# Lain-Iwakuro/Plonky2-Demo

Hardware: NVIDIA B200
Metric: lde_merkle_commit_elems_per_s (higher is better)
Workload: dtype u64 (Goldilocks field, integer)

## Files before the change

### plonky2_demo_b200/csrc/poseidon.cuh

```cuda
#pragma once
#include "gl64.cuh"
#include "poseidon_constants.cuh"

namespace pcs {

#ifndef PCS_MDS_FP64
#define PCS_MDS_FP64 1
#endif
#ifndef PCS_SBOX_GROUP
#define PCS_SBOX_GROUP 12
#endif

constexpr int SPONGE_WIDTH = 12;
constexpr int SPONGE_RATE = 8;

__device__ __forceinline__ uint64_t sbox7(uint64_t x) {
    uint64_t x2 = gl::sqr(x);
    uint64_t x4 = gl::sqr(x2);
    uint64_t x3 = gl::mul(x, x2);
    return gl::mul(x3, x4);
}

__device__ __forceinline__ void mds_half(const uint32_t (&s)[12], const uint32_t (&add)[12], uint64_t (&y)[12]) {
    int64_t A[3], B[3], P[3], Q[3];
#pragma unroll
    for (int j = 0; j < 3; j++) {
        int64_t s0 = s[j], s3 = s[j + 3], s6 = s[j + 6], s9 = s[j + 9];
        int64_t u = s0 + s6, v = s3 + s9;
        A[j] = u + v;
        B[j] = u - v;
        P[j] = s0 - s6;
        Q[j] = s3 - s9;
    }
    int64_t t = A[0] + A[1] + A[2];
    int64_t Ya[3] = {(t + A[2]) << 4, (t + A[0]) << 4, (t + A[1]) << 4};
    int64_t Yb[3] = {(B[2] << 3) - (B[1] << 1) - B[0],
                     -(B[0] << 3) - B[1] - (B[2] << 1),
                     (B[0] << 1) - (B[1] << 3) - B[2]};
    int64_t re[3], im[3];
    re[0] = (P[0] << 1) - Q[0] + P[1] - (Q[1] << 4) + P[2] + (Q[2] << 2);
    im[0] = P[0] + (Q[0] << 1) + (P[1] << 4) + Q[1] - (P[2] << 2) + Q[2];
    re[1] = -(P[0] << 2) + Q[0] + (P[1] << 1) - Q[1] + P[2] - (Q[2] << 4);
    im[1] = -P[0] - (Q[0] << 2) + P[1] + (Q[1] << 1) + (P[2] << 4) + Q[2];
    re[2] = (P[0] << 4) + Q[0] - (P[1] << 2) + Q[1] + (P[2] << 1) - Q[2];
    im[2] = -P[0] + (Q[0] << 4) - P[1] - (Q[1] << 2) + P[2] + (Q[2] << 1);
#pragma unroll
    for (int j = 0; j < 3; j++) {
        int64_t e1 = Ya[j] + Yb[j], e2 = Ya[j] - Yb[j];
        y[j] = (uint64_t)(e1 + re[j] + (int64_t)add[j]);
        y[j + 3] = (uint64_t)(e2 + im[j] + (int64_t)add[j + 3]);
        y[j + 6] = (uint64_t)(e1 - re[j] + (int64_t)add[j + 6]);
        y[j + 9] = (uint64_t)(e2 - im[j] + (int64_t)add[j + 9]);
    }
    y[0] += (uint64_t)s[0] << 3;
}

template <int RC_MODE >
__device__ __forceinline__ void mds_layer(uint64_t (&s)[12], const uint64_t* __restrict__ rc) {
    uint32_t lo[12], hi[12], alo[12], ahi[12];
#pragma unroll
    for (int i = 0; i < 12; i++) {
        lo[i] = (uint32_t)s[i];
        hi[i] = (uint32_t)(s[i] >> 32);
        uint64_t c = (RC_MODE == 1 || (RC_MODE == 2 && i == 0)) ? rc[i] : 0;
        alo[i] = (uint32_t)c;
        ahi[i] = (uint32_t)(c >> 32);
    }
    uint64_t L[12], H[12];
    mds_half(lo, alo, L);
    mds_half(hi, ahi, H);
#pragma unroll
    for (int r = 0; r < 12; r++) s[r] = gl::fold_halves(L[r], H[r]);
}

constexpr double TWO52 = 4503599627370496.0;

__device__ __forceinline__ void mds_half_fp64(const uint32_t (&s)[12], const double* __restrict__ addb ,
                                              uint32_t (&ylo)[12], uint32_t (&yhi)[12]) {
    double A[3], B[3], P[3], Q[3];
    double s0d;
#pragma unroll
    for (int j = 0; j < 3; j++) {
        double v0 = __hiloint2double(0x43300000, (int)s[j]), v3 = __hiloint2double(0x43300000, (int)s[j + 3]);
        double v6 = __hiloint2double(0x43300000, (int)s[j + 6]), v9 = __hiloint2double(0x43300000, (int)s[j + 9]);
        double d6 = v6 - TWO52, d9 = v9 - TWO52;
        P[j] = v0 - v6;
        Q[j] = v3 - v9;
        double u = fma(d6, 2.0, P[j]);
        double v = fma(d9, 2.0, Q[j]);
        A[j] = u + v;
        B[j] = u - v;
        if (j == 0) s0d = P[0] + d6;
    }
    double t = A[0] + A[1] + A[2];
    double Ya[3] = {t + A[2], t + A[0], t + A[1]};
    double Yb[3] = {fma(B[1], -2.0, fma(B[2], 8.0, -B[0])),
                    fma(B[2], -2.0, fma(B[0], -8.0, -B[1])),
                    fma(B[1], -8.0, fma(B[0], 2.0, -B[2]))};
    double re[3], im[3];
    re[0] = fma(Q[2], 4.0, fma(Q[1], -16.0, fma(P[0], 2.0, -Q[0]) + P[1]) + P[2]);
    im[0] = fma(P[2], -4.0, fma(P[1], 16.0, fma(Q[0], 2.0, P[0]) + Q[1]) + Q[2]);
    re[1] = fma(Q[2], -16.0, fma(P[1], 2.0, fma(P[0], -4.0, Q[0]) - Q[1]) + P[2]);
    im[1] = fma(P[2], 16.0, fma(Q[1], 2.0, fma(Q[0], -4.0, -P[0]) + P[1]) + Q[2]);
    re[2] = fma(P[2], 2.0, fma(P[1], -4.0, fma(P[0], 16.0, Q[0]) + Q[1]) - Q[2]);
    im[2] = fma(Q[2], 2.0, fma(Q[1], -4.0, fma(Q[0], 16.0, -P[0]) - P[1]) + P[2]);
#pragma unroll
    for (int j = 0; j < 3; j++) {
        double e1 = fma(Ya[j], 16.0, Yb[j]), e2 = fma(Ya[j], 16.0, -Yb[j]);
        double y0 = e1 + re[j];
        if (j == 0) y0 = fma(s0d, 8.0, y0);
        double r0 = y0 + addb[2 * j];
        double r3 = (e2 + im[j]) + addb[2 * (j + 3)];
        double r6 = (e1 - re[j]) + addb[2 * (j + 6)];
        double r9 = (e2 - im[j]) + addb[2 * (j + 9)];
        ylo[j] = (uint32_t)__double2loint(r0);     yhi[j] = (uint32_t)__double2hiint(r0);
        ylo[j + 3] = (uint32_t)__double2loint(r3); yhi[j + 3] = (uint32_t)__double2hiint(r3);
        ylo[j + 6] = (uint32_t)__double2loint(r6); yhi[j + 6] = (uint32_t)__double2hiint(r6);
        ylo[j + 9] = (uint32_t)__double2loint(r9); yhi[j + 9] = (uint32_t)__double2hiint(r9);
    }
}

__device__ __forceinline__ void mds_layer_fp64(uint64_t (&s)[12], const uint64_t* __restrict__ rcd) {
    const double* addb = reinterpret_cast<const double*>(rcd);
    uint32_t lo[12], hi[12];
#pragma unroll
    for (int i = 0; i < 12; i++) {
        lo[i] = (uint32_t)s[i];
        hi[i] = (uint32_t)(s[i] >> 32);
    }
    uint32_t l0[12], l1[12], h0[12], h1[12];
    mds_half_fp64(lo, addb, l0, l1);
    mds_half_fp64(hi, addb + 1, h0, h1);
#pragma unroll
    for (int r = 0; r < 12; r++) s[r] = gl::fold_halves_biased(l0[r], l1[r], h0[r], h1[r]);
}

__device__ __forceinline__ double u32_as_double(uint32_t x) { return __hiloint2double(0x43300000, (int)x) - TWO52; }

template <bool ZERO0>
__device__ __forceinline__ void mds_net_d(const double (&s)[12], double (&y)[12]) {
    double A[3], B[3], P[3], Q[3];
#pragma unroll
    for (int j = 0; j < 3; j++) {
        const bool z = ZERO0 && j == 0;
        double u = z ? s[6] : s[j] + s[j + 6], v = s[j + 3] + s[j + 9];
        A[j] = u + v;
        B[j] = u - v;
        P[j] = z ? -s[6] : s[j] - s[j + 6];
        Q[j] = s[j + 3] - s[j + 9];
    }
    double t = A[0] + A[1] + A[2];
    double Ya[3] = {t + A[2], t + A[0], t + A[1]};
    double Yb[3] = {fma(B[1], -2.0, fma(B[2], 8.0, -B[0])),
                    fma(B[2], -2.0, fma(B[0], -8.0, -B[1])),
                    fma(B[1], -8.0, fma(B[0], 2.0, -B[2]))};
    double re[3], im[3];
    re[0] = fma(Q[2], 4.0, fma(Q[1], -16.0, fma(P[0], 2.0, -Q[0]) + P[1]) + P[2]);
    im[0] = fma(P[2], -4.0, fma(P[1], 16.0, fma(Q[0], 2.0, P[0]) + Q[1]) + Q[2]);
    re[1] = fma(Q[2], -16.0, fma(P[1], 2.0, fma(P[0], -4.0, Q[0]) - Q[1]) + P[2]);
    im[1] = fma(P[2], 16.0, fma(Q[1], 2.0, fma(Q[0], -4.0, -P[0]) + P[1]) + Q[2]);
    re[2] = fma(P[2], 2.0, fma(P[1], -4.0, fma(P[0], 16.0, Q[0]) + Q[1]) - Q[2]);
    im[2] = fma(Q[2], 2.0, fma(Q[1], -4.0, fma(Q[0], 16.0, -P[0]) - P[1]) + P[2]);
#pragma unroll
    for (int j = 0; j < 3; j++) {
        double e1 = fma(Ya[j], 16.0, Yb[j]), e2 = fma(Ya[j], 16.0, -Yb[j]);
        y[j] = e1 + re[j];
        y[j + 3] = e2 + im[j];
        y[j + 6] = e1 - re[j];
        y[j + 9] = e2 - im[j];
    }
    if (!ZERO0) y[0] = fma(s[0], 8.0, y[0]);
}

__device__ __forceinline__ void renorm_d(double& lo, double& hi) {
    const double M1 = TWO52 + 1.0, INV32 = 1.0 / 4294967296.0;
    double l1m = __fma_rd(lo, INV32, TWO52) - M1;
    double h1m = __fma_rd(hi, INV32, TWO52) - M1;
    double lo2 = fma(l1m, -4294967296.0, lo) - h1m;
    double hi2 = fma(h1m, -4294967295.0, hi) + l1m;
    lo = lo2;
    hi = hi2;
}

__device__ __forceinline__ uint64_t fold_d(double lo, double hi) {
    double bl = lo + TWO52, bh = hi + TWO52;
    return gl::fold_halves_biased((uint32_t)__double2loint(bl), (uint32_t)__double2hiint(bl),
                                  (uint32_t)__double2loint(bh), (uint32_t)__double2hiint(bh));
}

#ifndef PCS_PARTIAL_SPLIT
#define PCS_PARTIAL_SPLIT 0
#endif
__device__ __forceinline__ void partial_round_d(uint64_t& x0, double (&dl)[12], double (&dh)[12], uint64_t rc) {
    double yl[12], yh[12];
#if PCS_PARTIAL_SPLIT
    mds_net_d<true>(dl, yl);
    mds_net_d<true>(dh, yh);
    x0 = gl::add_lc_p(sbox7(x0), rc);
    const double al = u32_as_double((uint32_t)x0), ah = u32_as_double((uint32_t)(x0 >> 32));
    constexpr double COL0[12] = {25.0, 20.0, 34.0, 18.0, 39.0, 13.0, 13.0, 28.0, 2.0, 16.0, 41.0, 15.0};
#pragma unroll
    for (int i = 0; i < 12; i++) {
        dl[i] = fma(al, COL0[i], yl[i]);
        dh[i] = fma(ah, COL0[i], yh[i]);
    }
#else
    x0 = gl::add_lc_p(sbox7(x0), rc);
    dl[0] = u32_as_double((uint32_t)x0);
    dh[0] = u32_as_double((uint32_t)(x0 >> 32));
    mds_net_d<false>(dl, yl);
    mds_net_d<false>(dh, yh);
#pragma unroll
    for (int i = 0; i < 12; i++) {
        dl[i] = yl[i];
        dh[i] = yh[i];
    }
#endif
}

#ifndef PCS_PARTIAL_FP64
#define PCS_PARTIAL_FP64 1
#endif

__device__ __forceinline__ void full_round(uint64_t (&s)[12], int r) {
    using namespace pconst;
#if PCS_SBOX_GROUP == 12
#pragma unroll
    for (int i = 0; i < 12; i++) s[i] = sbox7(s[i]);
#else
#pragma unroll 1
    for (int g = 0; g < 12 / PCS_SBOX_GROUP; g++) {
        uint64_t t[PCS_SBOX_GROUP];
#pragma unroll
        for (int i = 0; i < PCS_SBOX_GROUP; i++) t[i] = sbox7(s[i]);
#pragma unroll
        for (int i = 0; i < 12 - PCS_SBOX_GROUP; i++) s[i] = s[i + PCS_SBOX_GROUP];
#pragma unroll
        for (int i = 0; i < PCS_SBOX_GROUP; i++) s[12 - PCS_SBOX_GROUP + i] = t[i];
    }
#endif
#if PCS_MDS_FP64
    mds_layer_fp64(s, &ROUND_ADD_D[24 * r]);
#else
    mds_layer<1>(s, &ROUND_ADD[12 * r]);
#endif
}

template <bool CANON_OUT = true>
__device__ __forceinline__ void poseidon12(uint64_t (&s)[12]) {
    using namespace pconst;
#pragma unroll
    for (int i = 0; i < 12; i++) s[i] = gl::add_lc_p(s[i], RC[i]);
#if PCS_PARTIAL_FP64 && PCS_MDS_FP64
#pragma unroll 1
    for (int phase = 0; phase < 2; phase++) {
#pragma unroll 1
        for (int r = 0; r < 4; r++) full_round(s, 26 * phase + r);
        if (phase == 0) {
            uint64_t x0 = s[0];
            double dl[12], dh[12];
#pragma unroll
            for (int i = 1; i < 12; i++) {
                dl[i] = u32_as_double((uint32_t)s[i]);
                dh[i] = u32_as_double((uint32_t)(s[i] >> 32));
            }
#pragma unroll 1
            for (int k = 0; k < 11; k++) {
                partial_round_d(x0, dl, dh, PARTIAL_RC[2 * k]);
                x0 = fold_d(dl[0], dh[0]);
                partial_round_d(x0, dl, dh, PARTIAL_RC[2 * k + 1]);
                if (k < 10) {
                    x0 = fold_d(dl[0], dh[0]);
#pragma unroll
                    for (int i = 1; i < 12; i++) renorm_d(dl[i], dh[i]);
                }
            }
            const double* rcd = reinterpret_cast<const double*>(&ROUND_ADD_D[24 * 25]);
#pragma unroll
            for (int i = 0; i < 12; i++) {
                double bl = dl[i] + rcd[2 * i], bh = dh[i] + rcd[2 * i + 1];
                s[i] = gl::fold_halves_biased((uint32_t)__double2loint(bl), (uint32_t)__double2hiint(bl),
                                              (uint32_t)__double2loint(bh), (uint32_t)__double2hiint(bh));
            }
        }
    }
#else
#pragma unroll 1
    for (int r = 0; r < 30; r++) {
        if (r < 4 || r >= 26) {
#pragma unroll
            for (int i = 0; i < 12; i++) s[i] = sbox7(s[i]);
        } else {
            s[0] = sbox7(s[0]);
        }
#if PCS_MDS_FP64
        mds_layer_fp64(s, &ROUND_ADD_D[24 * r]);
#else
        mds_layer<1>(s, &ROUND_ADD[12 * r]);
#endif
    }
#endif
    if (CANON_OUT) {
#pragma unroll
        for (int i = 0; i < 12; i++) s[i] = gl::canon(s[i]);
    }
}

}
```

Baseline: 9.582 billion.

## Keep Poseidon partial-round state in a transformed (CRT-like) FP64 basis

Replaces the per-partial-round full MDS butterfly in FP64 with a state kept in a pre-transformed basis (forward/mid/scale stages). Each round then only updates lane 0 and runs a reduced mid-stage before converting back to output lanes at the end. Renormalization now uses a different magic constant that allows signed values, and a biased fold is applied to lane 0. The aim is fewer FP64 operations per partial round, at the cost of more intricate numeric range reasoning and a risk of exactness errors.

Measured after the change: 10.07 billion, median of 6. 5.1% higher.

```diff
diff --git a/plonky2_demo_b200/csrc/poseidon.cuh b/plonky2_demo_b200/csrc/poseidon.cuh
--- a/plonky2_demo_b200/csrc/poseidon.cuh
+++ b/plonky2_demo_b200/csrc/poseidon.cuh
@@ -136,6 +136,7 @@
 }
 
 __device__ __forceinline__ double u32_as_double(uint32_t x) { return __hiloint2double(0x43300000, (int)x) - TWO52; }
+__device__ __forceinline__ double u32_biased(uint32_t x) { return __hiloint2double(0x43300000, (int)x); }
 
 template <bool ZERO0>
 __device__ __forceinline__ void mds_net_d(const double (&s)[12], double (&y)[12]) {
@@ -172,50 +173,89 @@
     if (!ZERO0) y[0] = fma(s[0], 8.0, y[0]);
 }
 
+__device__ __forceinline__ void crt_forward_d(const uint32_t (&s)[12], double (&u)[12]) {
+#pragma unroll
+    for (int j = 0; j < 3; j++) {
+        double v0 = u32_biased(s[j]), v3 = u32_biased(s[j + 3]), v6 = u32_biased(s[j + 6]), v9 = u32_biased(s[j + 9]);
+        double P = v0 - v6, Q = v3 - v9;
+        double a = fma(v6 - TWO52, 2.0, P);
+        double b = fma(v9 - TWO52, 2.0, Q);
+        u[j] = a + b;
+        u[j + 3] = a - b;
+        u[j + 6] = P;
+        u[j + 9] = Q;
+    }
+}
+
+__device__ __forceinline__ void crt_mid_half(const double (&u)[12], double g, double (&w)[12]) {
+    const double A0 = u[0] + g, A1 = u[1], A2 = u[2];
+    const double B0 = u[3] + g, B1 = u[4], B2 = u[5];
+    const double P0 = u[6] + g, P1 = u[7], P2 = u[8];
+    const double Q0 = u[9], Q1 = u[10], Q2 = u[11];
+    const double T = ((A1 + A2) + A0) * 64.0;
+    w[0] = fma(A2, 64.0, T);
+    w[1] = fma(A0, 64.0, T);
+    w[2] = fma(A1, 64.0, T);
+    w[3] = fma(B1, -2.0, fma(B2, 8.0, -B0));
+    w[4] = fma(B2, -2.0, fma(B0, -8.0, -B1));
+    w[5] = fma(B1, -8.0, fma(B0, 2.0, -B2));
+    w[6] = fma(Q2, 4.0, fma(Q1, -16.0, fma(P0, 2.0, -Q0) + P1) + P2);
+    w[7] = fma(Q2, -16.0, fma(P1, 2.0, fma(P0, -4.0, Q0) - Q1) + P2);
+    w[8] = fma(P2, 2.0, fma(P1, -4.0, fma(P0, 16.0, Q0) + Q1) - Q2);
+    w[9] = fma(P2, -4.0, fma(P1, 16.0, fma(Q0, 2.0, P0) + Q1) + Q2);
+    w[10] = fma(P2, 16.0, fma(Q1, 2.0, fma(Q0, -4.0, -P0) + P1) + Q2);
+    w[11] = fma(Q2, 2.0, fma(Q1, -4.0, fma(Q0, 16.0, -P0) - P1) + P2);
+}
+
+__device__ __forceinline__ double crt_scale_half(const double (&w)[12], double (&u)[12]) {
+#pragma unroll
+    for (int j = 0; j < 3; j++) {
+        u[j] = w[j];
+        u[j + 3] = w[j + 3] * 4.0;
+        u[j + 6] = w[j + 6] * 2.0;
+        u[j + 9] = w[j + 9] * 2.0;
+    }
+    return fma(w[0], 0.25, w[3] + w[6]);
+}
+
+__device__ __forceinline__ void crt_lanes_half(const double (&w)[12], double bias, const double* __restrict__ rcd,
+                                               double (&y)[12]) {
+#pragma unroll
+    for (int j = 0; j < 3; j++) {
+        double e1 = fma(w[j], 0.25, w[j + 3] + bias), e2 = fma(w[j], 0.25, bias - w[j + 3]);
+        y[j] = (e1 + w[j + 6]) + rcd[2 * j];
+        y[j + 6] = (e1 - w[j + 6]) + rcd[2 * (j + 6)];
+        y[j + 3] = (e2 + w[j + 9]) + rcd[2 * (j + 3)];
+        y[j + 9] = (e2 - w[j + 9]) + rcd[2 * (j + 9)];
+    }
+}
+
 __device__ __forceinline__ void renorm_d(double& lo, double& hi) {
-    const double M1 = TWO52 + 1.0, INV32 = 1.0 / 4294967296.0;
-    double l1m = __fma_rd(lo, INV32, TWO52) - M1;
-    double h1m = __fma_rd(hi, INV32, TWO52) - M1;
-    double lo2 = fma(l1m, -4294967296.0, lo) - h1m;
-    double hi2 = fma(h1m, -4294967295.0, hi) + l1m;
+    const double C = 6755399441055744.0, INV32 = 1.0 / 4294967296.0;
+    double l1 = __fma_rd(lo, INV32, C) - C;
+    double h1 = __fma_rd(hi, INV32, C) - C;
+    double lo2 = fma(l1, -4294967296.0, lo) - h1;
+    double hi2 = fma(h1, -4294967295.0, hi) + l1;
     lo = lo2;
     hi = hi2;
 }
 
-__device__ __forceinline__ uint64_t fold_d(double lo, double hi) {
-    double bl = lo + TWO52, bh = hi + TWO52;
+constexpr double BIAS_LO = 2251799813685248.0 + 524288.0;
+constexpr double BIAS_HI = 2251799813685248.0 - 1048576.0;
+
+__device__ __forceinline__ uint64_t fold_signed_d(double lo, double hi) {
+    double bl = lo + (TWO52 + BIAS_LO), bh = hi + (TWO52 + BIAS_HI);
     return gl::fold_halves_biased((uint32_t)__double2loint(bl), (uint32_t)__double2hiint(bl),
                                   (uint32_t)__double2loint(bh), (uint32_t)__double2hiint(bh));
 }
 
-#ifndef PCS_PARTIAL_SPLIT
-#define PCS_PARTIAL_SPLIT 0
-#endif
-__device__ __forceinline__ void partial_round_d(uint64_t& x0, double (&dl)[12], double (&dh)[12], uint64_t rc) {
-    double yl[12], yh[12];
-#if PCS_PARTIAL_SPLIT
-    mds_net_d<true>(dl, yl);
-    mds_net_d<true>(dh, yh);
-    x0 = gl::add_lc_p(sbox7(x0), rc);
-    const double al = u32_as_double((uint32_t)x0), ah = u32_as_double((uint32_t)(x0 >> 32));
-    constexpr double COL0[12] = {25.0, 20.0, 34.0, 18.0, 39.0, 13.0, 13.0, 28.0, 2.0, 16.0, 41.0, 15.0};
-#pragma unroll
-    for (int i = 0; i < 12; i++) {
-        dl[i] = fma(al, COL0[i], yl[i]);
-        dh[i] = fma(ah, COL0[i], yh[i]);
-    }
-#else
-    x0 = gl::add_lc_p(sbox7(x0), rc);
-    dl[0] = u32_as_double((uint32_t)x0);
-    dh[0] = u32_as_double((uint32_t)(x0 >> 32));
-    mds_net_d<false>(dl, yl);
-    mds_net_d<false>(dh, yh);
-#pragma unroll
-    for (int i = 0; i < 12; i++) {
-        dl[i] = yl[i];
-        dh[i] = yh[i];
-    }
-#endif
+__device__ __forceinline__ void lane0_crt(double el, double eh, double& xl, double& xh, uint64_t rc, double& gl, double& gh) {
+    const uint64_t s0 = fold_signed_d(fma(xl, 8.0, el), fma(xh, 8.0, eh));
+    const uint64_t x = gl::add_lc_p(sbox7(s0), rc);
+    gl = fma(xl, 8.0, u32_biased((uint32_t)x) - u32_biased((uint32_t)s0));
+    gh = fma(xh, 8.0, u32_biased((uint32_t)(x >> 32)) - u32_biased((uint32_t)(s0 >> 32)));
+    xl = u32_as_double((uint32_t)x);
+    xh = u32_as_double((uint32_t)(x >> 32));
 }
 
 #ifndef PCS_PARTIAL_FP64
@@ -257,28 +297,46 @@
 #pragma unroll 1
         for (int r = 0; r < 4; r++) full_round(s, 26 * phase + r);
         if (phase == 0) {
-            uint64_t x0 = s[0];
-            double dl[12], dh[12];
-#pragma unroll
-            for (int i = 1; i < 12; i++) {
-                dl[i] = u32_as_double((uint32_t)s[i]);
-                dh[i] = u32_as_double((uint32_t)(s[i] >> 32));
+            double ul[12], uh[12];
+            {
+                uint32_t lo[12], hi[12];
+#pragma unroll
+                for (int i = 0; i < 12; i++) {
+                    lo[i] = (uint32_t)s[i];
+                    hi[i] = (uint32_t)(s[i] >> 32);
+                }
+                crt_forward_d(lo, ul);
+                crt_forward_d(hi, uh);
             }
+            double el = u32_as_double((uint32_t)s[0]), eh = u32_as_double((uint32_t)(s[0] >> 32));
+            double xl = 0.0, xh = 0.0;
+            const double* rcd = reinterpret_cast<const double*>(&ROUND_ADD_D[24 * 25]);
 #pragma unroll 1
             for (int k = 0; k < 11; k++) {
-                partial_round_d(x0, dl, dh, PARTIAL_RC[2 * k]);
-                x0 = fold_d(dl[0], dh[0]);
-                partial_round_d(x0, dl, dh, PARTIAL_RC[2 * k + 1]);
+                double gl, gh, wl[12], wh[12];
+                lane0_crt(el, eh, xl, xh, PARTIAL_RC[2 * k], gl, gh);
+                crt_mid_half(ul, gl, wl);
+                crt_mid_half(uh, gh, wh);
+                el = crt_scale_half(wl, ul);
+                eh = crt_scale_half(wh, uh);
+                lane0_crt(el, eh, xl, xh, PARTIAL_RC[2 * k + 1], gl, gh);
+                crt_mid_half(ul, gl, wl);
+                crt_mid_half(uh, gh, wh);
                 if (k < 10) {
-                    x0 = fold_d(dl[0], dh[0]);
-#pragma unroll
-                    for (int i = 1; i < 12; i++) renorm_d(dl[i], dh[i]);
+                    el = crt_scale_half(wl, ul);
+                    eh = crt_scale_half(wh, uh);
+#pragma unroll
+                    for (int i = 0; i < 12; i++) renorm_d(ul[i], uh[i]);
+                } else {
+                    crt_lanes_half(wl, BIAS_LO, rcd, ul);
+                    crt_lanes_half(wh, BIAS_HI, rcd + 1, uh);
+                    ul[0] = fma(xl, 8.0, ul[0]);
+                    uh[0] = fma(xh, 8.0, uh[0]);
                 }
             }
-            const double* rcd = reinterpret_cast<const double*>(&ROUND_ADD_D[24 * 25]);
 #pragma unroll
             for (int i = 0; i < 12; i++) {
-                double bl = dl[i] + rcd[2 * i], bh = dh[i] + rcd[2 * i + 1];
+                const double bl = ul[i], bh = uh[i];
                 s[i] = gl::fold_halves_biased((uint32_t)__double2loint(bl), (uint32_t)__double2hiint(bl),
                                               (uint32_t)__double2loint(bh), (uint32_t)__double2hiint(bh));
             }
```
